# ETM-Code/eirgrid

Hardware: NVIDIA B200
Metric: full 2025-2050 episodes simulated and scored per second (higher is better)
Workload: dtype f64

## Files before the change

### eirgrid_b200/_lib.py

```python
import ctypes as C
import os

import numpy as np

from . import _abi

HERE = os.path.dirname(os.path.abspath(__file__))
LIB_PATH = os.path.join(HERE, os.environ.get("EIRGRID_LIB_NAME", "libeirgrid_b200.so"))

EXPORTS = [
    "eg_init", "eg_destroy", "eg_last_error", "eg_sync", "eg_kernel_launches", "eg_map_load", "eg_map_set",
    "eg_map_info", "eg_map_site_tables", "eg_map_site_static", "eg_weights_new", "eg_weights_free",
    "eg_weights_clone", "eg_weights_load_json", "eg_weights_save_json", "eg_weights_merge", "eg_weights_get_table",
    "eg_weights_set_table", "eg_weights_get_best", "eg_deficit_key_action", "eg_rollout_batch", "eg_weights_upload",
    "eg_rollout_batch_device", "eg_replay_batch", "eg_replay_batch_device", "eg_update", "eg_update_stats_device",
    "eg_update_apply_stats", "eg_location_analysis", "eg_update_stats_clear_device", "eg_update_pack_best_device",
    "eg_location_analysis_year", "eg_microbench_fp64", "eg_export_best_run_csv", "eg_weights_history_append", "eg_train_batch_begin", "eg_train_batch_end", "eg_train_batch_results", "eg_update_combine_apply",
    "eg_update_device", "eg_train_batch_inorder", "eg_rule_math",
    "eg_location_analysis_sites", "eg_location_analysis_sites_device", "eg_location_analysis_write",
    "eg_update_pack_exchange_device",
]


class EirgridError(RuntimeError):
    def __init__(self, code, message):
        super().__init__("eirgrid_b200 error %d: %s" % (code, message))
        self.code = code


_lib = None


def lib():
    global _lib
    if _lib is not None:
        return _lib
    if not os.path.exists(LIB_PATH):
        raise ImportError("%s is missing: run `python -m eirgrid_b200.build` (needs nvcc). "
                          "eirgrid_b200 has no CPU fallback." % LIB_PATH)
    L = C.CDLL(LIB_PATH)
    vp, u32, u64, i64 = C.c_void_p, C.c_uint32, C.c_uint64, C.c_int64
    L.eg_last_error.restype = C.c_char_p
    L.eg_init.argtypes = [C.c_int, vp, C.POINTER(vp)]
# ... 11 lines not shown
    L.eg_weights_free.argtypes = [vp]
    L.eg_weights_free.restype = None
    L.eg_weights_clone.argtypes = [vp, C.POINTER(vp)]
    L.eg_weights_load_json.argtypes = [C.c_char_p, C.POINTER(vp)]
    L.eg_weights_save_json.argtypes = [vp, C.c_char_p]
    L.eg_weights_merge.argtypes = [vp, vp]
    L.eg_weights_get_table.argtypes = [vp, C.POINTER(_abi.WeightsTable)]
    L.eg_weights_set_table.argtypes = [vp, C.POINTER(_abi.WeightsTable)]
    L.eg_weights_get_best.argtypes = [vp, vp, vp, C.c_size_t, vp, vp, C.c_size_t]
    L.eg_deficit_key_action.argtypes = [u32]
    L.eg_deficit_key_action.restype = C.c_uint8
    L.eg_rollout_batch.argtypes = [vp, vp, C.POINTER(_abi.RunCfg), u64, u64, u32, vp, vp, vp, vp]
    L.eg_weights_upload.argtypes = [vp, vp]
    L.eg_rollout_batch_device.argtypes = [vp, C.POINTER(_abi.RunCfg), u64, u64, u32, vp, vp, vp, vp]
    L.eg_replay_batch.argtypes = [vp, C.POINTER(_abi.RunCfg), vp, u32, vp, vp, vp]
    L.eg_replay_batch_device.argtypes = [vp, C.POINTER(_abi.RunCfg), vp, u32, vp, vp, vp]
    L.eg_update.argtypes = [vp, vp, vp, u32, u32, u64, C.POINTER(_abi.UpdateStats)]
    L.eg_update_device.argtypes = [vp, vp, vp, vp, u32, u32, u64, C.POINTER(_abi.UpdateStats)]
    L.eg_train_batch_inorder.argtypes = [vp, vp, C.POINTER(_abi.RunCfg), u64, u64, u32, u64, C.POINTER(_abi.UpdateStats)]
    L.eg_update_stats_device.argtypes = [vp, vp, vp, vp, u32, vp, vp, vp]
    L.eg_update_stats_clear_device.argtypes = [vp, vp]
    L.eg_update_pack_exchange_device.argtypes = [vp, vp, vp, u32, vp, vp, vp, u64, vp, vp, u32, u32, u32, vp]
    L.eg_update_pack_best_device.argtypes = [vp, vp, vp, u32, vp, vp, u64, vp]
    L.eg_weights_history_append.argtypes = [vp, u64, C.c_char_p]
    L.eg_location_analysis_sites.argtypes = [vp, C.c_int, u32, C.c_double, u32, u32, u32, u32, vp]
    L.eg_location_analysis_sites_device.argtypes = [vp, C.c_int, u32, C.c_double, u32, u32, u32, u32, vp]
    L.eg_location_analysis_write.argtypes = [vp, C.c_int, C.c_double, C.c_char_p, C.c_char_p]
    L.eg_rule_math.argtypes = [C.c_int, u32, vp, vp, u32, vp]
    L.eg_microbench_fp64.argtypes = [C.c_int, C.POINTER(C.c_double)]
    L.eg_export_best_run_csv.argtypes = [vp, vp, C.POINTER(_abi.RunCfg), C.c_char_p, C.c_char_p]
    L.eg_train_batch_begin.argtypes = [vp, vp, C.POINTER(_abi.RunCfg), u64, u64, u32]
    L.eg_train_batch_end.argtypes = [vp, vp, vp]
    L.eg_train_batch_results.argtypes = [vp, vp, vp]
    L.eg_update_combine_apply.argtypes = [vp, vp, vp, u32, u64, u64, C.POINTER(_abi.UpdateStats)]
    L.eg_update_apply_stats.argtypes = [vp, vp, u64, vp, vp, i64, C.POINTER(_abi.UpdateStats)]
    L.eg_location_analysis.argtypes = [vp, C.c_int, C.c_int32, C.c_double, vp, u32, u32]
    L.eg_location_analysis_year.argtypes = [vp, C.c_int, u32, C.c_int32, C.c_double, vp, u32, u32]
    _lib = L
    return L


def check(rc):
    if rc < 0:
        raise EirgridError(rc, lib().eg_last_error().decode("utf-8", "replace"))
    return rc

# ... 189 lines not shown
        st = _abi.UpdateStats()
        check(self.L.eg_update_device(self.h, weights.h, _dev_ptr(d_results), _dev_ptr(d_traj), int(n), int(replay_best),
                                      int(rng_seed), C.byref(st)))
        return st

    def train_batch_inorder(self, weights, n, seed, first_episode, cfg=None, rng_seed=0):
        cfg = cfg or _abi.RunCfg()
        st = _abi.UpdateStats()
        check(self.L.eg_train_batch_inorder(self.h, weights.h, C.byref(cfg), int(seed), int(first_episode), int(n),
                                            int(rng_seed), C.byref(st)))
        return st

    def update_stats_device(self, weights, n, d_results, d_traj, d_stats, d_best_score, d_best_index):
        check(self.L.eg_update_stats_device(self.h, weights.h, _dev_ptr(d_results), _dev_ptr(d_traj), n,
                                            _dev_ptr(d_stats), _dev_ptr(d_best_score), _dev_ptr(d_best_index)))

    def update_stats_clear_device(self, d_stats):
        check(self.L.eg_update_stats_clear_device(self.h, _dev_ptr(d_stats)))

    def update_pack_best_device(self, n, d_results, d_traj, d_best_score, d_best_index, first_global_episode, d_record):
        check(self.L.eg_update_pack_best_device(self.h, _dev_ptr(d_results), _dev_ptr(d_traj), n, _dev_ptr(d_best_score),
                                                _dev_ptr(d_best_index), first_global_episode, _dev_ptr(d_record)))

    def update_pack_exchange_device(self, n, d_results, d_traj, d_stats, d_best_score, d_best_index, first_global_episode,
                                    peer_buffers, peer_flags, rank, epoch, d_error):
        world = len(peer_buffers)
        pb = (C.c_uint64 * world)(*[int(x) for x in peer_buffers])
        pf = (C.c_uint64 * world)(*[int(x) for x in peer_flags])
        check(self.L.eg_update_pack_exchange_device(self.h, _dev_ptr(d_results), _dev_ptr(d_traj), n, _dev_ptr(d_stats),
                                                    _dev_ptr(d_best_score), _dev_ptr(d_best_index), int(first_global_episode),
                                                    pb, pf, world, int(rank), int(epoch), _dev_ptr(d_error)))

    def export_best_run_csv(self, weights, output_dir, cfg=None):
        cfg = cfg or _abi.RunCfg()
        buf = C.create_string_buffer(512)
        check(self.L.eg_export_best_run_csv(self.h, weights.h, C.byref(cfg), os.fsencode(output_dir), buf))
        return buf.value.decode()

    def location_analysis(self, use_loaded_map, half_steps=25, step=2000.0, first_point=0, n_points=None, year_index=0):
        side = 2 * half_steps + 1
        n = side * side - first_point if n_points is None else n_points
        out = np.zeros((n, _abi.N_GEN_TYPES))
        check(self.L.eg_location_analysis_year(self.h, int(use_loaded_map), int(year_index), half_steps, step, _abi.ptr(out), first_point, n))
        return out

    def location_analysis_sites(self, use_loaded_map, sites_per_axis, step, year_first=0, n_years=26, first_site=0, n_sites=None,
# ... 28 lines not shown
```

### eirgrid_b200/csrc/engine.cu

```cuda
#include <cuda_runtime.h>
#include <cmath>
#include <sys/stat.h>
#include <sys/types.h>
#include <cstdio>
#include <cstdlib>
#include <cstring>
#include <ctime>
#include <string>
#include <vector>
#include "common.hpp"
#include "episode.cuh"
#include "host_tables.hpp"
#include "json_min.hpp"
#include "site_tables.cuh"
#include "stats.cuh"
#include "suitability.cuh"
#include "update.cuh"
#include "weights.hpp"

static_assert(sizeof(EgPolicyDevice) == 38784, "bench.py and eirgrid_b200/_abi.py quote this size");
static thread_local std::string g_last_error;
int eg_fail(int code, const std::string& message) {
  g_last_error = message;
  return code;
// ... 24 lines not shown
  double* d_prefix = nullptr;
  double* d_static_unsorted = nullptr;
  uint16_t* d_order = nullptr;
  double* d_static_sorted = nullptr;
  double* d_prefix_sorted = nullptr;
  double* d_walk = nullptr;
  double* d_near = nullptr;
  int* d_r2_limit = nullptr;
  double *d_sx = nullptr, *d_sy = nullptr, *d_ex = nullptr, *d_ey = nullptr, *d_cx = nullptr, *d_cy = nullptr;
  uint32_t* d_pop = nullptr;
  double* d_suit_rows = nullptr;
  size_t suit_rows_cap = 0;
  double* d_urban_r = nullptr;
  double urban_r_max = 0.0;
  EgPolicyDevice* d_policy = nullptr;
  EgPolicyDevice* h_policy[2] = {nullptr, nullptr};
  cudaEvent_t policy_copied[2] = {nullptr, nullptr};
  int policy_turn = 0;
  uint32_t* d_next_episode = nullptr;
  int64_t* d_stats = nullptr;
  double* d_best_score = nullptr;
  unsigned long long* d_best_index = nullptr;
  unsigned char* d_record = nullptr;
  int64_t* h_stats = nullptr;
  unsigned char* h_record = nullptr;
  uint32_t train_n = 0;
  bool train_pending = false;
  EgUpdBuffers upd{};
  EgUpdState* h_upd_state = nullptr;
  EgUpdSlot* h_upd_slot = nullptr;
  EgUpdImprovement* h_upd_imp = nullptr;
  EgDeviceMap dmap{};
  size_t cap = 0;
  eg_result* s_out = nullptr;
  eg_traj* s_traj = nullptr;
  eg_traj* s_traj_in = nullptr;
  eg_sites* s_sites = nullptr;
  eg_yearly* s_yearly = nullptr;
  size_t cap_yearly = 0, cap_sites = 0, cap_traj_in = 0;
};

namespace {

void free_map(eg_ctx* c) {
  void* ptrs[] = {c->d_small, c->d_plant_terms, c->d_site_opinion, c->d_coast, c->d_prefix, c->d_static_unsorted, c->d_order,
                  c->d_static_sorted, c->d_prefix_sorted, c->d_walk, c->d_near, c->d_r2_limit, c->d_sx, c->d_sy, c->d_ex, c->d_ey, c->d_cx, c->d_cy, c->d_pop, c->d_urban_r};
// ... 173 lines not shown
  if (e3 != cudaSuccess) { if (c->own_stream) cudaStreamDestroy(c->stream); delete c; return eg_fail(EG_ERR_CUDA, cudaGetErrorString(e3)); }
  *out = c;
  return EG_OK;
}

void eg_destroy(eg_ctx* c) {
  if (!c) return;
  cudaSetDevice(c->device);
  cudaStreamSynchronize(c->stream);
  free_map(c);
  if (c->h_stats) cudaFreeHost(c->h_stats);
  if (c->h_record) cudaFreeHost(c->h_record);
  for (int b = 0; b < 2; b++) {
    if (c->h_policy[b]) cudaFreeHost(c->h_policy[b]);
    if (c->policy_copied[b]) cudaEventDestroy(c->policy_copied[b]);
  }
  if (c->h_upd_state) cudaFreeHost(c->h_upd_state);
  if (c->h_upd_slot) cudaFreeHost(c->h_upd_slot);
  if (c->h_upd_imp) cudaFreeHost(c->h_upd_imp);
  if (c->d_suit_rows) cudaFree(c->d_suit_rows);
  void* upd_ptrs[] = {c->upd.state, c->upd.slots, c->upd.score, c->upd.pre, c->upd.ctl, c->upd.counts, c->upd.factors, c->upd.improvements};
  for (void* p : upd_ptrs)
    if (p) cudaFree(p);
  void* ptrs[] = {c->d_policy, c->d_next_episode, c->d_stats, c->d_best_score, c->d_best_index, c->d_record, c->s_out, c->s_traj, c->s_traj_in, c->s_sites, c->s_yearly};
  for (void* p : ptrs)
    if (p) cudaFree(p);
  if (c->own_stream) cudaStreamDestroy(c->stream);
  delete c;
}

int eg_sync(eg_ctx* c) {
  if (!c) return eg_fail(EG_ERR_INVALID, "ctx is NULL");
  EG_CUDA(cudaStreamSynchronize(c->stream));
  return EG_OK;
}

uint64_t eg_kernel_launches(const eg_ctx* c) { return c ? c->launches : 0; }

int eg_map_load(eg_ctx* c, const char* settlements_json, const char* generators_csv, const char* coastline_json) {
  if (!c || !settlements_json || !generators_csv || !coastline_json) return eg_fail(EG_ERR_INVALID, "eg_map_load: NULL argument");
  int rc = eg_host_map_load(&c->hmap, settlements_json, generators_csv, coastline_json);
  if (rc) return rc;
  return build_device_map(c);
}

int eg_map_set(eg_ctx* c, const eg_map_desc* desc) {
  if (!c) return eg_fail(EG_ERR_INVALID, "eg_map_set: ctx is NULL");
// ... 112 lines not shown
  p.replay_in = d_in;
  p.out = d_out; p.traj = nullptr; p.sites = d_sites; p.yearly = d_yearly;
  EG_CUDA(eg_launch_replay(p, c->stream));
  if (n) c->launches++;
  return EG_OK;
}

int eg_replay_batch(eg_ctx* c, const eg_run_cfg* cfg, const eg_traj* in, uint32_t n, eg_result* out, eg_sites* sites_out,
                    eg_yearly* yearly_out) {
  int rc = check_cfg(c, cfg);
  if (rc) return rc;
  if (!in || !out) return eg_fail(EG_ERR_INVALID, "eg_replay_batch: NULL argument");
  if ((rc = ensure_scratch(c, n, sites_out != nullptr, yearly_out != nullptr, true))) return rc;
  EG_CUDA(cudaMemcpyAsync(c->s_traj_in, in, (size_t)n * sizeof(eg_traj), cudaMemcpyHostToDevice, c->stream));
  rc = eg_replay_batch_device(c, cfg, c->s_traj_in, n, c->s_out, sites_out ? c->s_sites : nullptr, yearly_out ? c->s_yearly : nullptr);
  if (rc) return rc;
  EG_CUDA(cudaMemcpyAsync(out, c->s_out, (size_t)n * sizeof(eg_result), cudaMemcpyDeviceToHost, c->stream));
  if (sites_out) EG_CUDA(cudaMemcpyAsync(sites_out, c->s_sites, (size_t)n * sizeof(eg_sites), cudaMemcpyDeviceToHost, c->stream));
  if (yearly_out) EG_CUDA(cudaMemcpyAsync(yearly_out, c->s_yearly, (size_t)n * sizeof(eg_yearly), cudaMemcpyDeviceToHost, c->stream));
  EG_CUDA(cudaStreamSynchronize(c->stream));
  return EG_OK;
}

int eg_update_stats_device(eg_ctx* c, const eg_weights* w, const eg_result* d_results, const eg_traj* d_trajs, uint32_t n,
                           int64_t* d_stats, double* d_best_score, unsigned long long* d_best_index) {
  if (!c || !w || !d_results || !d_trajs || !d_stats || !d_best_score || !d_best_index)
    return eg_fail(EG_ERR_INVALID, "eg_update_stats_device: NULL argument");
  if (!c->policy_ready) return eg_fail(EG_ERR_STATE, "no weights uploaded: call eg_weights_upload first");
  EG_CUDA(cudaSetDevice(c->device));
  EgStatsParams p{};
  p.consts = eg_contrast_consts(*w);
  p.policy = c->d_policy;
  p.results = d_results; p.trajs = d_trajs; p.n = n;
  p.stats = d_stats; p.best_score = d_best_score; p.best_index = d_best_index;
  p.ln100 = std::log(50000000000.0 * 100.0 / 50000000000.0);
  EG_CUDA(eg_launch_stats(p, c->stream));
  c->launches += n ? 3 : 1;
  return EG_OK;
}

int eg_update_stats_clear_device(eg_ctx* c, int64_t* d_stats) {
  if (!c || !d_stats) return eg_fail(EG_ERR_INVALID, "eg_update_stats_clear_device: NULL argument");
  EG_CUDA(cudaSetDevice(c->device));
  EG_CUDA(cudaMemsetAsync(d_stats, 0, (size_t)EG_STATS_WORDS * sizeof(int64_t), c->stream));
  return EG_OK;
}

int eg_update_pack_best_device(eg_ctx* c, const eg_result* d_results, const eg_traj* d_trajs, uint32_t n, const double* d_best_score,
                               const unsigned long long* d_best_index, uint64_t first_global_episode, void* d_record) {
  if (!c || !d_results || !d_trajs || !d_best_score || !d_best_index || !d_record)
    return eg_fail(EG_ERR_INVALID, "eg_update_pack_best_device: NULL argument");
  EG_CUDA(cudaSetDevice(c->device));
  EG_CUDA(eg_launch_pack_best(d_results, d_trajs, n, d_best_score, d_best_index, first_global_episode, d_record, c->stream));
  c->launches++;
  return EG_OK;
}

int eg_update_pack_exchange_device(eg_ctx* c, const eg_result* d_results, const eg_traj* d_trajs, uint32_t n, const int64_t* d_stats,
                                   const double* d_best_score, const unsigned long long* d_best_index, uint64_t first_global_episode,
                                   const uint64_t* peer_buffers, const uint64_t* peer_flags, uint32_t world, uint32_t rank, uint32_t epoch,
                                   uint32_t* d_error) {
// ... 8 lines not shown
  EG_CUDA(eg_launch_pack_exchange(p, c->stream));
  c->launches++;
  return EG_OK;
}

int eg_train_batch_begin(eg_ctx* c, const eg_weights* w, const eg_run_cfg* cfg, uint64_t seed, uint64_t first_episode, uint32_t n) {
  int rc = check_cfg(c, cfg);
  if (rc) return rc;
  if (!w) return eg_fail(EG_ERR_INVALID, "eg_train_batch_begin: weights are NULL");
  if (c->train_pending) return eg_fail(EG_ERR_STATE, "eg_train_batch_begin: a batch is already in flight on this context");
  EG_CUDA(cudaSetDevice(c->device));
  if (!c->d_stats) {
    EG_CUDA(cudaMalloc((void**)&c->d_stats, EG_STATS_WORDS * sizeof(int64_t)));
    EG_CUDA(cudaMalloc((void**)&c->d_best_score, sizeof(double)));
    EG_CUDA(cudaMalloc((void**)&c->d_best_index, sizeof(unsigned long long)));
    EG_CUDA(cudaMalloc((void**)&c->d_record, EG_BEST_RECORD_BYTES));
    EG_CUDA(cudaMallocHost((void**)&c->h_stats, EG_STATS_WORDS * sizeof(int64_t)));
    EG_CUDA(cudaMallocHost((void**)&c->h_record, EG_BEST_RECORD_BYTES));
  }
  if ((rc = eg_weights_upload(c, w))) return rc;
  if ((rc = ensure_scratch(c, n, false, false, false))) return rc;
  if ((rc = eg_rollout_batch_device(c, cfg, seed, first_episode, n, c->s_out, c->s_traj, nullptr, nullptr))) return rc;
  if ((rc = eg_update_stats_clear_device(c, c->d_stats))) return rc;
  if ((rc = eg_update_stats_device(c, w, c->s_out, c->s_traj, n, c->d_stats, c->d_best_score, c->d_best_index))) return rc;
  if ((rc = eg_update_pack_best_device(c, c->s_out, c->s_traj, n, c->d_best_score, c->d_best_index, first_episode, c->d_record))) return rc;
  EG_CUDA(cudaMemcpyAsync(c->h_stats, c->d_stats, EG_STATS_WORDS * sizeof(int64_t), cudaMemcpyDeviceToHost, c->stream));
  EG_CUDA(cudaMemcpyAsync(c->h_record, c->d_record, EG_BEST_RECORD_BYTES, cudaMemcpyDeviceToHost, c->stream));
  c->train_n = n;
  c->train_pending = true;
  return EG_OK;
}

int eg_train_batch_end(eg_ctx* c, int64_t* stats_out, void* record_out) {
  if (!c || !stats_out || !record_out) return eg_fail(EG_ERR_INVALID, "eg_train_batch_end: NULL argument");
  if (!c->train_pending) return eg_fail(EG_ERR_STATE, "eg_train_batch_end: no batch in flight");
  EG_CUDA(cudaSetDevice(c->device));
  c->train_pending = false;
  EG_CUDA(cudaStreamSynchronize(c->stream));
  std::memcpy(stats_out, c->h_stats, EG_STATS_WORDS * sizeof(int64_t));
  std::memcpy(record_out, c->h_record, EG_BEST_RECORD_BYTES);
  return EG_OK;
}

int eg_train_batch_results(eg_ctx* c, eg_result* out, eg_traj* traj_out) {
  if (!c || !out) return eg_fail(EG_ERR_INVALID, "eg_train_batch_results: NULL argument");
  if (c->train_pending || !c->train_n) return eg_fail(EG_ERR_STATE, "eg_train_batch_results: no finished batch");
  EG_CUDA(cudaSetDevice(c->device));
  EG_CUDA(cudaMemcpyAsync(out, c->s_out, (size_t)c->train_n * sizeof(eg_result), cudaMemcpyDeviceToHost, c->stream));
// ... 534 lines not shown
```

### eirgrid_b200/csrc/stats.cu

```cuda
#include "stats.cuh"
#include <algorithm>

namespace {

constexpr double kMaxAcceptableCost = 50000000000.0, kMaxAcceptableEmissions = 1000000.0;

__device__ __forceinline__ double default_score(const eg_result& r, double ln100, bool cost_only = false) {
  if (cost_only) return 2.0 - fmin(log(fmax(r.total_cost / kMaxAcceptableCost, 1.0)) / ln100, 1.0);
  if (r.net_emissions > 0.0) return 1.0 - fmin(r.net_emissions / kMaxAcceptableEmissions, 1.0);
  const double normalized_cost = fmax(r.total_cost / kMaxAcceptableCost, 1.0);
  const double cost_score = 1.0 - fmin(log(normalized_cost) / ln100, 1.0);
  const double cost_weight = normalized_cost > 8.0 ? 0.8 : 0.5;
  return 1.0 + (cost_score * cost_weight + r.public_opinion * (1.0 - cost_weight));
}

__device__ __forceinline__ int deficit_key_of_action(int code) {
  if (code == EG_ACT_DO_NOTHING) return 14;
  if (code >= 45 || code % 3) return -1;
  switch (code / 3) {
    case 8: return 0; case 7: return 1; case 12: return 2; case 11: return 3; case 9: return 4; case 0: return 5;
    case 1: return 6; case 4: return 7; case 10: return 8; case 5: return 9; case 2: return 10; case 3: return 11;
    case 13: return 12; case 14: return 13;
  }
  return -1;
}

__global__ void eg_stats_reset_kernel(double* best_score, unsigned long long* best_index) {
  *best_score = -1.0;
  *best_index = ~0ull;
}

__global__ void __launch_bounds__(256) eg_stats_kernel(const EgStatsParams p) {
  __shared__ unsigned long long acc[EG_STATS_WORDS];
  __shared__ unsigned long long best_mask[EG_NY];
  __shared__ uint8_t best_cat[EG_BEST_CAPACITY + EG_TRAJ_CAPACITY];
  __shared__ uint16_t best_len[EG_NY], best_start[EG_NY];
  for (int i = threadIdx.x; i < EG_STATS_WORDS; i += blockDim.x) acc[i] = 0ull;
  if (threadIdx.x < EG_NY) {
    const int y = threadIdx.x;
    const int nb = p.policy->n_best[y], nbd = p.policy->n_best_deficit[y];
    const int ob = p.policy->best_off[y], obd = p.policy->best_deficit_off[y];
    uint8_t* cat = best_cat + ob + obd;
    unsigned long long m = 0ull;
    for (int b = 0; b < nb; b++) { const int a = p.policy->best[ob + b]; cat[b] = (uint8_t)a; m |= 1ull << a; }
    for (int b = 0; b < nbd; b++) { const int a = p.policy->best_deficit[obd + b]; cat[nb + b] = (uint8_t)a; m |= 1ull << a; }
    best_mask[y] = m;
    best_len[y] = (uint16_t)(nb + nbd);
    best_start[y] = (uint16_t)(ob + obd);
  }
  __syncthreads();
  const int lane = threadIdx.x & 31;
  const uint32_t warps_total = gridDim.x * (blockDim.x >> 5);
  double warp_best = -1.0;
  for (uint32_t ep = blockIdx.x * (blockDim.x >> 5) + (threadIdx.x >> 5); ep < p.n; ep += warps_total) {
    const eg_result* rp = p.results + ep;
    eg_result r;
    r.net_emissions = rp->net_emissions; r.public_opinion = rp->public_opinion; r.total_cost = rp->total_cost;
    const double score = default_score(r, p.ln100, p.consts.cost_only != 0);
    warp_best = fmax(warp_best, score);
    bool pass = false;
    long long log_pen = 0, log_mild = 0;
    if (p.consts.has_best) {
      const double det = p.consts.best_score > 0.0 ? (p.consts.best_score - score) / p.consts.best_score : 0.0;
      pass = det > p.consts.threshold || p.consts.force;
      if (pass) {
        if (det < 0.0) {
          log_pen = log_mild = -(1ll << 40);
        } else {
          const double combined = pow(det, 0.3) * p.consts.stagnation;
          const double penalty = 1.0 / (1.0 + p.consts.alr * 1.5 * combined);
          const double mild = 1.0 / (1.0 + p.consts.alr * combined * 0.5);
          log_pen = llrint(log(penalty) * EG_STATS_FIXED_SCALE);
          log_mild = llrint(log(mild) * EG_STATS_FIXED_SCALE);
        }
      }
    }
    if (lane == 0) {
      atomicAdd(&acc[0], 1ull);
      if (pass) atomicAdd(&acc[1], 1ull);
      if (rp->flags) atomicAdd(&acc[2], 1ull);
    }
    const eg_traj* t = p.trajs + ep;
    int nd = 0, nrun = 0;
    if (lane < EG_NY) { nd = t->n_deficit[lane]; nrun = nd + t->n_additional[lane]; }
    int row_end = nrun;
#pragma unroll
    for (int o = 1; o < 32; o <<= 1) {
      const int v = __shfl_up_sync(0xFFFFFFFFu, row_end, o);
      if (lane >= o) row_end += v;
    }
    int row = row_end - nrun;
    if (row > EG_TRAJ_CAPACITY) row = EG_TRAJ_CAPACITY;
    if (row + nrun > EG_TRAJ_CAPACITY) { nrun = EG_TRAJ_CAPACITY - row; nd = min(nd, nrun); }
    const int cnt = nrun + nd;
    int incl = cnt;
#pragma unroll
    for (int o = 1; o < 32; o <<= 1) {
      const int v = __shfl_up_sync(0xFFFFFFFFu, incl, o);
      if (lane >= o) incl += v;
    }
    const int total = __shfl_sync(0xFFFFFFFFu, incl, 31);
    for (int base = 0; base < total; base += 32) {
      const int q = base + lane;
      int y = 0;
#pragma unroll
      for (int step = 16; step > 0; step >>= 1) {
        const int v = __shfl_sync(0xFFFFFFFFu, incl, y + step - 1);
        if (v <= q) y += step;
      }
      const int y_incl = __shfl_sync(0xFFFFFFFFu, incl, y), y_cnt = __shfl_sync(0xFFFFFFFFu, cnt, y);
      const int y_nrun = __shfl_sync(0xFFFFFFFFu, nrun, y), y_row = __shfl_sync(0xFFFFFFFFu, row, y);
      if (q >= total) continue;
      const int i = q - (y_incl - y_cnt);
      const int a = t->actions[y_row + (i < y_nrun ? i : i - y_nrun)];
      if (a >= EG_N_ACTIONS) continue;
      unsigned long long* ys = acc + EG_STATS_HEADER + y * EG_STATS_YEAR_STRIDE;
      if (i < y_nrun) atomicAdd(&ys[2 * EG_N_ACTIONS + a], 1ull);
      else {
        const int k = deficit_key_of_action(a);
        if (k >= 0) atomicAdd(&ys[3 * EG_N_ACTIONS + k], 1ull);
      }
      if (!pass) continue;
      if (!((best_mask[y] >> a) & 1ull)) {
        atomicAdd(&ys[a], (unsigned long long)log_pen);
      } else if (i < (int)best_len[y]) {
        if (best_cat[best_start[y] + i] != a) atomicAdd(&ys[EG_N_ACTIONS + a], (unsigned long long)log_mild);
      }
    }
  }
  if (lane == 0 && warp_best >= 0.0) atomicMax((long long*)p.best_score, __double_as_longlong(warp_best));
  __syncthreads();
  for (int i = threadIdx.x; i < EG_STATS_WORDS; i += blockDim.x)
    if (acc[i]) atomicAdd((unsigned long long*)&p.stats[i], acc[i]);
}

__global__ void __launch_bounds__(256) eg_stats_argbest_kernel(const EgStatsParams p) {
  const uint32_t ep = blockIdx.x * blockDim.x + threadIdx.x;
  if (ep >= p.n) return;
  const double score = default_score(p.results[ep], p.ln100, p.consts.cost_only != 0);
  if (score == *p.best_score) atomicMin(p.best_index, (unsigned long long)ep);
}

__global__ void __launch_bounds__(320) eg_stats_pack_best_kernel(const eg_result* results, const eg_traj* trajs, uint32_t n, const double* best_score,
                                                                 const unsigned long long* best_index, unsigned long long first_global, uint32_t* record) {
  const unsigned long long raw = *best_index;
  const uint32_t idx = raw < n ? (uint32_t)raw : (n ? n - 1 : 0);
  const int w = threadIdx.x;
  constexpr int kRes = (int)sizeof(eg_result) / 4, kTraj = (int)sizeof(eg_traj) / 4;
  if (w < 2) record[w] = ((const uint32_t*)best_score)[w];
  else if (w < 4) { const unsigned long long g = first_global + idx; record[w] = (uint32_t)(g >> (32 * (w - 2))); }
  else if (w < 4 + kRes) record[w] = ((const uint32_t*)(results + idx))[w - 4];
  else if (w < 4 + kRes + kTraj) record[w] = ((const uint32_t*)(trajs + idx))[w - 4 - kRes];
}

__global__ void __launch_bounds__(256) eg_pack_exchange_kernel(const EgExchangeParams p) {
  constexpr int kRec = (int)(EG_BEST_RECORD_BYTES / 8), kWords = EG_STATS_WORDS + kRec;
  constexpr int kRes = (int)sizeof(eg_result) / 8;
  const uint32_t peer = blockIdx.x;
  const unsigned long long raw = *p.best_index;
  const uint32_t idx = raw < p.n ? (uint32_t)raw : (p.n ? p.n - 1 : 0);
  long long* dst = (long long*)p.peer_buf[peer] + ((size_t)(p.epoch & 1u) * p.world + p.rank) * kWords;
  const long long* res = (const long long*)(p.results + idx);
  const long long* trj = (const long long*)(p.trajs + idx);
  for (int i = threadIdx.x; i < kWords; i += blockDim.x) {
    long long v;
    if (i < EG_STATS_WORDS) v = p.stats[i];
    else {
      const int w = i - EG_STATS_WORDS;
      v = w == 0 ? __double_as_longlong(*p.best_score) : w == 1 ? (long long)(p.first_global + idx) : w < 2 + kRes ? res[w - 2] : trj[w - 2 - kRes];
    }
    dst[i] = v;
  }
  __threadfence_system();
  __syncthreads();
  if (threadIdx.x == 0) {
// ... 6 lines not shown
      asm volatile("ld.acquire.sys.global.u32 %0, [%1];" : "=r"(v) : "l"(mine) : "memory");
      if ((int32_t)(v - p.epoch) >= 0) break;
      if (clock64() - t0 > 4000000000ll) { *p.error = 1u; break; }
    }
  }
}

}

cudaError_t eg_launch_pack_exchange(const EgExchangeParams& p, cudaStream_t stream) {
  static_assert(EG_BEST_RECORD_BYTES % 8 == 0 && sizeof(eg_result) % 8 == 0 && sizeof(eg_traj) % 8 == 0, "the record is copied in 64-bit words");
  if (p.world == 0 || p.world > EG_MAX_PEERS || p.rank >= p.world) return cudaErrorInvalidValue;
  eg_pack_exchange_kernel<<<p.world, 256, 0, stream>>>(p);
  return cudaGetLastError();
}

cudaError_t eg_launch_pack_best(const eg_result* results, const eg_traj* trajs, uint32_t n, const double* best_score,
                                const unsigned long long* best_index, unsigned long long first_global, void* record, cudaStream_t stream) {
  static_assert(sizeof(eg_result) % 4 == 0 && sizeof(eg_traj) % 4 == 0, "record is copied in 32-bit words");
  eg_stats_pack_best_kernel<<<1, 320, 0, stream>>>(results, trajs, n, best_score, best_index, first_global, (uint32_t*)record);
  return cudaGetLastError();
}

cudaError_t eg_launch_stats(const EgStatsParams& p, cudaStream_t stream) {
  eg_stats_reset_kernel<<<1, 1, 0, stream>>>(p.best_score, p.best_index);
  if (p.n == 0) return cudaGetLastError();
  const uint32_t blocks = (p.n + 255) / 256;
  int dev = 0, sms = 148;
  cudaGetDevice(&dev);
  cudaDeviceGetAttribute(&sms, cudaDevAttrMultiProcessorCount, dev);
  const uint32_t stat_blocks = std::min<uint32_t>((uint32_t)sms * 4u, (p.n + 7) / 8);
  eg_stats_kernel<<<stat_blocks, 256, 0, stream>>>(p);
  eg_stats_argbest_kernel<<<blocks, 256, 0, stream>>>(p);
  return cudaGetLastError();
}
```

### eirgrid_b200/csrc/stats.cuh

```cuda
#pragma once
#include <cuda_runtime.h>
#include "tables.h"
#include "weights.hpp"

struct EgStatsParams {
  EgContrastConsts consts;
  const EgPolicyDevice* policy;
  const eg_result* results;
  const eg_traj* trajs;
  uint32_t n;
  int64_t* stats;
  double* best_score;
  unsigned long long* best_index;
  double ln100;
};

cudaError_t eg_launch_pack_best(const eg_result* results, const eg_traj* trajs, uint32_t n, const double* best_score,
                                const unsigned long long* best_index, unsigned long long first_global, void* record, cudaStream_t stream);

cudaError_t eg_launch_stats(const EgStatsParams& p, cudaStream_t stream);

#define EG_MAX_PEERS 16
struct EgExchangeParams {
  const eg_result* results;
  const eg_traj* trajs;
  uint32_t n;
  const double* best_score;
  const unsigned long long* best_index;
  unsigned long long first_global;
  const int64_t* stats;
  unsigned long long peer_buf[EG_MAX_PEERS];
  unsigned long long peer_flag[EG_MAX_PEERS];
  uint32_t world, rank, epoch;
  uint32_t* error;
};
cudaError_t eg_launch_pack_exchange(const EgExchangeParams& p, cudaStream_t stream);
```

### eirgrid_b200/trainer.py

```python
import ctypes as C
import os

import numpy as np

from . import _abi, _lib


def _torch():
    import torch
    return torch


REC_BYTES = 16 + _abi.RESULT_DTYPE.itemsize + _abi.TRAJ_DTYPE.itemsize
assert REC_BYTES % 8 == 0


def pack_record(score, global_index, result, traj):
    rec = np.zeros(REC_BYTES, np.uint8)
    rec[0:8] = np.frombuffer(np.float64(score).tobytes(), np.uint8)
    rec[8:16] = np.frombuffer(np.int64(global_index).tobytes(), np.uint8)
    rb = _abi.RESULT_DTYPE.itemsize
    rec[16:16 + rb] = np.frombuffer(np.ascontiguousarray(result).tobytes(), np.uint8)
    rec[16 + rb:] = np.frombuffer(np.ascontiguousarray(traj).tobytes(), np.uint8)
    return rec
# ... 48 lines not shown
        assert self.stream.cuda_stream != 0
        if map_arrays is not None:
            self.ctx.map_set(*map_arrays)
        else:
            self.ctx.map_load_dir(asset_dir)
        self.n = int(episodes_per_gpu)
        self.seed = int(seed)
        self.cfg = cfg or _abi.RunCfg()
        self.weights = weights or _lib.Weights()
        self.next_episode = 0
        self.offset = self.rank * self.n
        self.n_total = self.n * self.world
        u8 = torch.uint8
        self.d_results = torch.empty(self.n * _abi.RESULT_DTYPE.itemsize, dtype=u8, device=self.device)
        self.d_traj = torch.empty(self.n * _abi.TRAJ_DTYPE.itemsize, dtype=u8, device=self.device)
        self.d_sites = torch.empty(self.n * _abi.SITES_DTYPE.itemsize, dtype=u8, device=self.device) if want_sites else None
        self.rec_bytes = REC_BYTES
        self.pack_words = PACK_WORDS
        self.d_pack = torch.zeros(self.pack_words, dtype=torch.int64, device=self.device)
        self.d_stats = self.d_pack[:_abi.STATS_WORDS]
        self.d_rec = self.d_pack[_abi.STATS_WORDS:].view(u8)
        self.d_best_score = torch.zeros(1, dtype=torch.float64, device=self.device)
        self.d_best_index = torch.zeros(1, dtype=torch.int64, device=self.device)
        self.d_all_pack = torch.zeros(self.world * self.pack_words, dtype=torch.int64, device=self.device)
        self.h_all_pack = torch.zeros(self.world * self.pack_words, dtype=torch.int64).pin_memory()
        self.h2d_bytes_per_step = 0
        self.d2h_bytes_per_step = self.h_all_pack.numel() * 8
        self._init_peer_exchange()
        self.last_stats = None
        torch.cuda.synchronize(self.device)

    def _init_peer_exchange(self):
        torch = _torch()
        self.peer = None
        self.exchange_kind = "none" if self.world == 1 else "nccl all-gather"
        if not (self.dist and self.world > 1):
            return
        ok, peer = 1, None
        if os.environ.get("EIRGRID_EXCHANGE", "peer") != "peer":
            ok = 0
        else:
            try:
                import torch.distributed._symmetric_memory as symm
                buf = symm.empty(2 * self.world * self.pack_words, dtype=torch.int64, device=self.device)
                hdl = symm.rendezvous(buf, self.dist.group.WORLD)
                flags = symm.empty(64, dtype=torch.int32, device=self.device)
                fhdl = symm.rendezvous(flags, self.dist.group.WORLD)
# ... 11 lines not shown
        torch.cuda.synchronize(self.device)
        if int(agree.item()) == 1:
            self.peer = peer
            self.epoch = 0
            self.d_error = torch.zeros(1, dtype=torch.int32, device=self.device)
            self.exchange_kind = "one kernel over NVLink peer memory (symmetric allocation)"
            self.dist.barrier()
            torch.cuda.synchronize(self.device)

    def set_batch(self, total):
        self.offset, self.n = shard_of(total, self.rank, self.world)
        assert self.n <= self.d_results.numel() // _abi.RESULT_DTYPE.itemsize, "batch larger than the buffers"
        self.n_total = int(total)

    def upload_weights(self):
        self.ctx.weights_upload(self.weights)

    def launch_rollout(self, first_episode=None):
        first = self.next_episode + self.offset if first_episode is None else first_episode
        self.ctx.rollout_device(self.n, self.seed, first, self.d_results, self.d_traj, self.d_sites, None, self.cfg)

    def launch_stats(self):
        self.ctx.update_stats_clear_device(self.d_stats)
        self.ctx.update_stats_device(self.weights, self.n, self.d_results, self.d_traj, self.d_stats, self.d_best_score,
                                     self.d_best_index)

    def _pack_best(self):
        self.ctx.update_pack_best_device(self.n, self.d_results, self.d_traj, self.d_best_score, self.d_best_index,
                                         self.next_episode + self.offset, self.d_rec)

    def exchange(self):
        if self.peer is not None:
            self.epoch += 1
            self.ctx.update_pack_exchange_device(self.n, self.d_results, self.d_traj, self.d_stats, self.d_best_score, self.d_best_index,
                                                 self.next_episode + self.offset, self.peer["buf_ptrs"], self.peer["flag_ptrs"], self.rank,
                                                 self.epoch, self.d_error)
            half = (self.epoch & 1) * self.world * self.pack_words
            self.d_all_pack = self.peer["buf"][half:half + self.world * self.pack_words]
            return
        self._pack_best()
        with _torch().cuda.stream(self.stream):
            if self.dist and self.world > 1:
                self.dist.all_gather_into_tensor(self.d_all_pack, self.d_pack)
            else:
                self.d_all_pack.copy_(self.d_pack)

    def reduce_stats(self):
        self.exchange()

    def check_exchange(self):
        if self.peer is not None and int(self.d_error.item()) != 0:
            raise _lib.EirgridError(-3, "exchange step: a peer rank did not deliver its statistics within 2 s")

    def warm_exchange(self):
        self.exchange()
        with _torch().cuda.stream(self.stream):
            self.h_all_pack.copy_(self.d_all_pack, non_blocking=True)
        self.stream.synchronize()

    def step(self):
        torch = _torch()
        self.upload_weights()
        self.launch_rollout()
        self.launch_stats()
        self.exchange()
        with torch.cuda.stream(self.stream):
            self.h_all_pack.copy_(self.d_all_pack, non_blocking=True)
        self.stream.synchronize()
# ... 51 lines not shown
```

### include/eirgrid_b200.h

```cpp
#ifndef EIRGRID_B200_H
#define EIRGRID_B200_H

#include <stddef.h>
#include <stdint.h>

#ifdef __cplusplus
extern "C" {
#endif

#define EG_BASE_YEAR 2025
#define EG_END_YEAR 2050
#define EG_N_YEARS 26
#define EG_N_GEN_TYPES 15
#define EG_N_OFFSET_TYPES 4
#define EG_N_MULTS 3
#define EG_N_ACTIONS 61
#define EG_N_DEFICIT_KEYS 15
#define EG_N_COUNT_KEYS 21
#define EG_TRAJ_CAPACITY 984
#define EG_BEST_CAPACITY (2 * EG_TRAJ_CAPACITY)
#define EG_SITE_NONE 0xFFFFu

#define EG_ACT_UPGRADE 57
#define EG_ACT_ADJUST 58
// ... 158 lines not shown
int eg_replay_batch(eg_ctx* ctx, const eg_run_cfg* cfg, const eg_traj* in, uint32_t n, eg_result* out,
                    eg_sites* sites_out, eg_yearly* yearly_out);
int eg_replay_batch_device(eg_ctx* ctx, const eg_run_cfg* cfg, const eg_traj* d_in, uint32_t n,
                           eg_result* d_out, eg_sites* d_sites, eg_yearly* d_yearly);

int eg_update(eg_weights* w, const eg_result* results, const eg_traj* trajs, uint32_t n,
              uint32_t replay_best, uint64_t rng_seed, eg_update_stats* stats_out);

int eg_update_device(eg_ctx* ctx, eg_weights* w, const eg_result* d_results, const eg_traj* d_trajs, uint32_t n,
                     uint32_t replay_best, uint64_t rng_seed, eg_update_stats* stats_out);
int eg_train_batch_inorder(eg_ctx* ctx, eg_weights* w, const eg_run_cfg* cfg, uint64_t seed, uint64_t first_episode, uint32_t n,
                           uint64_t rng_seed, eg_update_stats* stats_out);

#define EG_STATS_WORDS (8 + EG_N_YEARS * (3 * EG_N_ACTIONS + EG_N_DEFICIT_KEYS))
int eg_update_stats_device(eg_ctx* ctx, const eg_weights* w, const eg_result* d_results, const eg_traj* d_trajs, uint32_t n,
                           int64_t* d_stats ,
                           double* d_best_score ,
                           unsigned long long* d_best_index );
int eg_update_stats_clear_device(eg_ctx* ctx, int64_t* d_stats);
#define EG_BEST_RECORD_BYTES (16 + sizeof(eg_result) + sizeof(eg_traj))
int eg_update_pack_best_device(eg_ctx* ctx, const eg_result* d_results, const eg_traj* d_trajs, uint32_t n,
                               const double* d_best_score, const unsigned long long* d_best_index,
                               uint64_t first_global_episode, void* d_record);
int eg_update_pack_exchange_device(eg_ctx* ctx, const eg_result* d_results, const eg_traj* d_trajs, uint32_t n, const int64_t* d_stats,
                                   const double* d_best_score, const unsigned long long* d_best_index, uint64_t first_global_episode,
                                   const uint64_t* peer_buffers, const uint64_t* peer_flags, uint32_t world, uint32_t rank,
                                   uint32_t epoch, uint32_t* d_error);
int eg_update_apply_stats(eg_weights* w, const int64_t* stats, uint64_t n_total,
                          const eg_result* batch_best_result, const eg_traj* batch_best_traj,
                          int64_t batch_best_index, eg_update_stats* stats_out);

int eg_train_batch_begin(eg_ctx* ctx, const eg_weights* w, const eg_run_cfg* cfg, uint64_t seed, uint64_t first_episode, uint32_t n);
int eg_train_batch_end(eg_ctx* ctx, int64_t* stats_out, void* record_out);
int eg_train_batch_results(eg_ctx* ctx, eg_result* out, eg_traj* traj_out );
int eg_update_combine_apply(eg_weights* w, const int64_t* stats_sum, const void* records, uint32_t n_records,
                            uint64_t n_total, uint64_t first_episode, eg_update_stats* stats_out);

int eg_export_best_run_csv(eg_ctx* ctx, const eg_weights* w, const eg_run_cfg* cfg, const char* output_dir, char* written_dir);

int eg_location_analysis(eg_ctx* ctx, int use_loaded_map, int32_t half_steps, double step,
                         double* scores_out, uint32_t first_point, uint32_t n_points);
int eg_location_analysis_year(eg_ctx* ctx, int use_loaded_map, uint32_t year_index, int32_t half_steps, double step,
                              double* scores_out, uint32_t first_point, uint32_t n_points);

int eg_location_analysis_sites(eg_ctx* ctx, int use_loaded_map, uint32_t sites_per_axis, double step, uint32_t year_first,
                               uint32_t n_years, uint32_t first_site, uint32_t n_sites, double* scores_out);
// ... 12 lines not shown
```

Measured before the change: 20.43 million.

## Fuse stats reset, argbest and best-record packing into one stats kernel

Replaces the reset, stats and argbest kernels plus the separate pack-best kernel with a single stats kernel. It tracks per-warp best score and index, reduces them per block, and uses a last-block ticket to pick the global best and write the record. It also prefetches the next episode's loads, reads actions through warp shuffles of a preloaded word, and skips the single-GPU device copy of the pack buffer. The cost removed is several launches and full extra passes over results. In exchange it adds a grid-wide ticket that relies on threadfence ordering and a persistent scratch buffer.

New measurement: 20.51 million (median of 6 runs). Within noise of the previous version (+0.4%).

```diff
diff --git a/eirgrid_b200/_lib.py b/eirgrid_b200/_lib.py
--- a/eirgrid_b200/_lib.py
+++ b/eirgrid_b200/_lib.py
@@ -18,7 +18,7 @@
     "eg_location_analysis_year", "eg_microbench_fp64", "eg_export_best_run_csv", "eg_weights_history_append", "eg_train_batch_begin", "eg_train_batch_end", "eg_train_batch_results", "eg_update_combine_apply",
     "eg_update_device", "eg_train_batch_inorder", "eg_rule_math",
     "eg_location_analysis_sites", "eg_location_analysis_sites_device", "eg_location_analysis_write",
-    "eg_update_pack_exchange_device",
+    "eg_update_pack_exchange_device", "eg_update_stats_pack_device",
 ]
 
 
@@ -76,6 +76,7 @@
     L.eg_update_stats_clear_device.argtypes = [vp, vp]
     L.eg_update_pack_exchange_device.argtypes = [vp, vp, vp, u32, vp, vp, vp, u64, vp, vp, u32, u32, u32, vp]
     L.eg_update_pack_best_device.argtypes = [vp, vp, vp, u32, vp, vp, u64, vp]
+    L.eg_update_stats_pack_device.argtypes = [vp, vp, vp, vp, u32, vp, vp, vp, u64, vp]
     L.eg_weights_history_append.argtypes = [vp, u64, C.c_char_p]
     L.eg_location_analysis_sites.argtypes = [vp, C.c_int, u32, C.c_double, u32, u32, u32, u32, vp]
     L.eg_location_analysis_sites_device.argtypes = [vp, C.c_int, u32, C.c_double, u32, u32, u32, u32, vp]
@@ -311,6 +312,12 @@
         check(self.L.eg_update_pack_best_device(self.h, _dev_ptr(d_results), _dev_ptr(d_traj), n, _dev_ptr(d_best_score),
                                                 _dev_ptr(d_best_index), first_global_episode, _dev_ptr(d_record)))
 
+    def update_stats_pack_device(self, weights, n, d_results, d_traj, d_stats, d_best_score, d_best_index, first_global_episode,
+                                 d_record):
+        check(self.L.eg_update_stats_pack_device(self.h, weights.h, _dev_ptr(d_results), _dev_ptr(d_traj), n, _dev_ptr(d_stats),
+                                                 _dev_ptr(d_best_score), _dev_ptr(d_best_index), first_global_episode,
+                                                 _dev_ptr(d_record)))
+
     def update_pack_exchange_device(self, n, d_results, d_traj, d_stats, d_best_score, d_best_index, first_global_episode,
                                     peer_buffers, peer_flags, rank, epoch, d_error):
         world = len(peer_buffers)
diff --git a/eirgrid_b200/csrc/engine.cu b/eirgrid_b200/csrc/engine.cu
--- a/eirgrid_b200/csrc/engine.cu
+++ b/eirgrid_b200/csrc/engine.cu
@@ -70,6 +70,7 @@
   double* d_best_score = nullptr;
   unsigned long long* d_best_index = nullptr;
   unsigned char* d_record = nullptr;
+  unsigned long long* d_stats_scratch = nullptr;
   int64_t* h_stats = nullptr;
   unsigned char* h_record = nullptr;
   uint32_t train_n = 0;
@@ -289,7 +290,7 @@
   void* upd_ptrs[] = {c->upd.state, c->upd.slots, c->upd.score, c->upd.pre, c->upd.ctl, c->upd.counts, c->upd.factors, c->upd.improvements};
   for (void* p : upd_ptrs)
     if (p) cudaFree(p);
-  void* ptrs[] = {c->d_policy, c->d_next_episode, c->d_stats, c->d_best_score, c->d_best_index, c->d_record, c->s_out, c->s_traj, c->s_traj_in, c->s_sites, c->s_yearly};
+  void* ptrs[] = {c->d_policy, c->d_next_episode, c->d_stats, c->d_best_score, c->d_best_index, c->d_record, c->d_stats_scratch, c->s_out, c->s_traj, c->s_traj_in, c->s_sites, c->s_yearly};
   for (void* p : ptrs)
     if (p) cudaFree(p);
   if (c->own_stream) cudaStreamDestroy(c->stream);
@@ -448,21 +449,42 @@
   return EG_OK;
 }
 
-int eg_update_stats_device(eg_ctx* c, const eg_weights* w, const eg_result* d_results, const eg_traj* d_trajs, uint32_t n,
-                           int64_t* d_stats, double* d_best_score, unsigned long long* d_best_index) {
-  if (!c || !w || !d_results || !d_trajs || !d_stats || !d_best_score || !d_best_index)
-    return eg_fail(EG_ERR_INVALID, "eg_update_stats_device: NULL argument");
+static int launch_stats(eg_ctx* c, const eg_weights* w, const eg_result* d_results, const eg_traj* d_trajs, uint32_t n, int64_t* d_stats,
+                        double* d_best_score, unsigned long long* d_best_index, uint64_t first_global_episode, void* d_record) {
   if (!c->policy_ready) return eg_fail(EG_ERR_STATE, "no weights uploaded: call eg_weights_upload first");
   EG_CUDA(cudaSetDevice(c->device));
+  if (!c->d_stats_scratch) {
+    size_t words = 0;
+    EG_CUDA(eg_stats_scratch_words(&words));
+    EG_CUDA(cudaMalloc((void**)&c->d_stats_scratch, words * sizeof(unsigned long long)));
+    EG_CUDA(cudaMemsetAsync(c->d_stats_scratch, 0, words * sizeof(unsigned long long), c->stream));
+  }
   EgStatsParams p{};
   p.consts = eg_contrast_consts(*w);
   p.policy = c->d_policy;
   p.results = d_results; p.trajs = d_trajs; p.n = n;
   p.stats = d_stats; p.best_score = d_best_score; p.best_index = d_best_index;
   p.ln100 = std::log(50000000000.0 * 100.0 / 50000000000.0);
+  p.first_global = first_global_episode; p.record = (uint32_t*)d_record;
+  p.scratch = c->d_stats_scratch;
   EG_CUDA(eg_launch_stats(p, c->stream));
-  c->launches += n ? 3 : 1;
-  return EG_OK;
+  c->launches++;
+  return EG_OK;
+}
+
+int eg_update_stats_device(eg_ctx* c, const eg_weights* w, const eg_result* d_results, const eg_traj* d_trajs, uint32_t n,
+                           int64_t* d_stats, double* d_best_score, unsigned long long* d_best_index) {
+  if (!c || !w || !d_results || !d_trajs || !d_stats || !d_best_score || !d_best_index)
+    return eg_fail(EG_ERR_INVALID, "eg_update_stats_device: NULL argument");
+  return launch_stats(c, w, d_results, d_trajs, n, d_stats, d_best_score, d_best_index, 0, nullptr);
+}
+
+int eg_update_stats_pack_device(eg_ctx* c, const eg_weights* w, const eg_result* d_results, const eg_traj* d_trajs, uint32_t n,
+                                int64_t* d_stats, double* d_best_score, unsigned long long* d_best_index, uint64_t first_global_episode,
+                                void* d_record) {
+  if (!c || !w || !d_results || !d_trajs || !d_stats || !d_best_score || !d_best_index || !d_record)
+    return eg_fail(EG_ERR_INVALID, "eg_update_stats_pack_device: NULL argument");
+  return launch_stats(c, w, d_results, d_trajs, n, d_stats, d_best_score, d_best_index, first_global_episode, d_record);
 }
 
 int eg_update_stats_clear_device(eg_ctx* c, int64_t* d_stats) {
@@ -517,8 +539,8 @@
   if ((rc = ensure_scratch(c, n, false, false, false))) return rc;
   if ((rc = eg_rollout_batch_device(c, cfg, seed, first_episode, n, c->s_out, c->s_traj, nullptr, nullptr))) return rc;
   if ((rc = eg_update_stats_clear_device(c, c->d_stats))) return rc;
-  if ((rc = eg_update_stats_device(c, w, c->s_out, c->s_traj, n, c->d_stats, c->d_best_score, c->d_best_index))) return rc;
-  if ((rc = eg_update_pack_best_device(c, c->s_out, c->s_traj, n, c->d_best_score, c->d_best_index, first_episode, c->d_record))) return rc;
+  if ((rc = eg_update_stats_pack_device(c, w, c->s_out, c->s_traj, n, c->d_stats, c->d_best_score, c->d_best_index, first_episode,
+                                        c->d_record))) return rc;
   EG_CUDA(cudaMemcpyAsync(c->h_stats, c->d_stats, EG_STATS_WORDS * sizeof(int64_t), cudaMemcpyDeviceToHost, c->stream));
   EG_CUDA(cudaMemcpyAsync(c->h_record, c->d_record, EG_BEST_RECORD_BYTES, cudaMemcpyDeviceToHost, c->stream));
   c->train_n = n;
diff --git a/eirgrid_b200/csrc/stats.cu b/eirgrid_b200/csrc/stats.cu
--- a/eirgrid_b200/csrc/stats.cu
+++ b/eirgrid_b200/csrc/stats.cu
@@ -2,6 +2,8 @@
 #include <algorithm>
 
 namespace {
+
+constexpr int kStatsThreads = 256, kStatsBlocksPerSm = 4, kTicketWords = 2;
 
 constexpr double kMaxAcceptableCost = 50000000000.0, kMaxAcceptableEmissions = 1000000.0;
 
@@ -25,16 +27,33 @@
   return -1;
 }
 
-__global__ void eg_stats_reset_kernel(double* best_score, unsigned long long* best_index) {
-  *best_score = -1.0;
-  *best_index = ~0ull;
-}
-
-__global__ void __launch_bounds__(256) eg_stats_kernel(const EgStatsParams p) {
+__device__ __forceinline__ bool better(double s, unsigned long long i, double bs, unsigned long long bi) {
+  return s > bs || (s == bs && i < bi);
+}
+
+__device__ __forceinline__ void write_record(const eg_result* results, const eg_traj* trajs, uint32_t n, double score,
+                                             unsigned long long raw, unsigned long long first_global, uint32_t* record, int t, int nt) {
+  constexpr int kRes = (int)sizeof(eg_result) / 4, kTraj = (int)sizeof(eg_traj) / 4;
+  const uint32_t idx = raw < n ? (uint32_t)raw : (n ? n - 1 : 0);
+  const unsigned long long bits = (unsigned long long)__double_as_longlong(score), g = first_global + idx;
+  for (int w = t; w < 4 + kRes + kTraj; w += nt) {
+    uint32_t v;
+    if (w < 2) v = (uint32_t)(bits >> (32 * w));
+    else if (w < 4) v = (uint32_t)(g >> (32 * (w - 2)));
+    else if (w < 4 + kRes) v = ((const uint32_t*)(results + idx))[w - 4];
+    else v = ((const uint32_t*)(trajs + idx))[w - 4 - kRes];
+    record[w] = v;
+  }
+}
+
+__global__ void __launch_bounds__(kStatsThreads, kStatsBlocksPerSm) eg_stats_kernel(const EgStatsParams p) {
   __shared__ unsigned long long acc[EG_STATS_WORDS];
   __shared__ unsigned long long best_mask[EG_NY];
   __shared__ uint8_t best_cat[EG_BEST_CAPACITY + EG_TRAJ_CAPACITY];
   __shared__ uint16_t best_len[EG_NY], best_start[EG_NY];
+  __shared__ double warp_best_s[kStatsThreads / 32];
+  __shared__ unsigned long long warp_best_i[kStatsThreads / 32];
+  __shared__ int last;
   for (int i = threadIdx.x; i < EG_STATS_WORDS; i += blockDim.x) acc[i] = 0ull;
   if (threadIdx.x < EG_NY) {
     const int y = threadIdx.x;
@@ -49,15 +68,33 @@
     best_start[y] = (uint16_t)(ob + obd);
   }
   __syncthreads();
-  const int lane = threadIdx.x & 31;
+  const int lane = threadIdx.x & 31, warp = threadIdx.x >> 5;
   const uint32_t warps_total = gridDim.x * (blockDim.x >> 5);
   double warp_best = -1.0;
-  for (uint32_t ep = blockIdx.x * (blockDim.x >> 5) + (threadIdx.x >> 5); ep < p.n; ep += warps_total) {
+  unsigned long long warp_best_ep = ~0ull;
+  struct Loads {
+    double net, opinion, cost;
+    uint32_t flags, act4;
+    int nd, nadd;
+  };
+  const auto load = [&](uint32_t ep, Loads& l) {
     const eg_result* rp = p.results + ep;
+    const eg_traj* t = p.trajs + ep;
+    l.net = rp->net_emissions; l.opinion = rp->public_opinion; l.cost = rp->total_cost; l.flags = rp->flags;
+    l.act4 = ((const uint32_t*)t->actions)[lane];
+    l.nd = lane < EG_NY ? t->n_deficit[lane] : 0;
+    l.nadd = lane < EG_NY ? t->n_additional[lane] : 0;
+  };
+  uint32_t ep = blockIdx.x * (blockDim.x >> 5) + warp;
+  Loads cur{};
+  if (ep < p.n) load(ep, cur);
+  for (; ep < p.n; ep += warps_total) {
+    Loads next{};
+    if (ep + warps_total < p.n) load(ep + warps_total, next);
     eg_result r;
-    r.net_emissions = rp->net_emissions; r.public_opinion = rp->public_opinion; r.total_cost = rp->total_cost;
+    r.net_emissions = cur.net; r.public_opinion = cur.opinion; r.total_cost = cur.cost;
     const double score = default_score(r, p.ln100, p.consts.cost_only != 0);
-    warp_best = fmax(warp_best, score);
+    if (score > warp_best) { warp_best = score; warp_best_ep = ep; }
     bool pass = false;
     long long log_pen = 0, log_mild = 0;
     if (p.consts.has_best) {
@@ -78,11 +115,9 @@
     if (lane == 0) {
       atomicAdd(&acc[0], 1ull);
       if (pass) atomicAdd(&acc[1], 1ull);
-      if (rp->flags) atomicAdd(&acc[2], 1ull);
-    }
-    const eg_traj* t = p.trajs + ep;
-    int nd = 0, nrun = 0;
-    if (lane < EG_NY) { nd = t->n_deficit[lane]; nrun = nd + t->n_additional[lane]; }
+      if (cur.flags) atomicAdd(&acc[2], 1ull);
+    }
+    int nd = cur.nd, nrun = cur.nd + cur.nadd;
     int row_end = nrun;
 #pragma unroll
     for (int o = 1; o < 32; o <<= 1) {
@@ -110,9 +145,11 @@
       }
       const int y_incl = __shfl_sync(0xFFFFFFFFu, incl, y), y_cnt = __shfl_sync(0xFFFFFFFFu, cnt, y);
       const int y_nrun = __shfl_sync(0xFFFFFFFFu, nrun, y), y_row = __shfl_sync(0xFFFFFFFFu, row, y);
+      const int i = q - (y_incl - y_cnt);
+      const int slot = q < total ? y_row + (i < y_nrun ? i : i - y_nrun) : 0;
+      const uint32_t word = __shfl_sync(0xFFFFFFFFu, cur.act4, (slot >> 2) & 31);
       if (q >= total) continue;
-      const int i = q - (y_incl - y_cnt);
-      const int a = t->actions[y_row + (i < y_nrun ? i : i - y_nrun)];
+      const int a = slot < 128 ? (int)((word >> (8 * (slot & 3))) & 0xFFu) : p.trajs[ep].actions[slot];
       if (a >= EG_N_ACTIONS) continue;
       unsigned long long* ys = acc + EG_STATS_HEADER + y * EG_STATS_YEAR_STRIDE;
       if (i < y_nrun) atomicAdd(&ys[2 * EG_N_ACTIONS + a], 1ull);
@@ -127,30 +164,57 @@
         if (best_cat[best_start[y] + i] != a) atomicAdd(&ys[EG_N_ACTIONS + a], (unsigned long long)log_mild);
       }
     }
-  }
-  if (lane == 0 && warp_best >= 0.0) atomicMax((long long*)p.best_score, __double_as_longlong(warp_best));
+    cur = next;
+  }
+  if (lane == 0) { warp_best_s[warp] = warp_best; warp_best_i[warp] = warp_best_ep; }
+
   __syncthreads();
   for (int i = threadIdx.x; i < EG_STATS_WORDS; i += blockDim.x)
     if (acc[i]) atomicAdd((unsigned long long*)&p.stats[i], acc[i]);
-}
-
-__global__ void __launch_bounds__(256) eg_stats_argbest_kernel(const EgStatsParams p) {
-  const uint32_t ep = blockIdx.x * blockDim.x + threadIdx.x;
-  if (ep >= p.n) return;
-  const double score = default_score(p.results[ep], p.ln100, p.consts.cost_only != 0);
-  if (score == *p.best_score) atomicMin(p.best_index, (unsigned long long)ep);
+  unsigned int* ticket = (unsigned int*)p.scratch;
+  unsigned long long* block_best = p.scratch + kTicketWords;
+  if (threadIdx.x == 0) {
+    double bs = warp_best_s[0];
+    unsigned long long bi = warp_best_i[0];
+    for (int w = 1; w < kStatsThreads / 32; w++)
+      if (better(warp_best_s[w], warp_best_i[w], bs, bi)) { bs = warp_best_s[w]; bi = warp_best_i[w]; }
+    block_best[2 * blockIdx.x] = (unsigned long long)__double_as_longlong(bs);
+    block_best[2 * blockIdx.x + 1] = bi;
+    __threadfence();
+    last = atomicAdd(ticket, 1u) == gridDim.x - 1;
+  }
+  __syncthreads();
+  if (!last) return;
+  __threadfence();
+  if (warp == 0) {
+    double bs = -1.0;
+    unsigned long long bi = ~0ull;
+    for (uint32_t b = lane; b < gridDim.x; b += 32) {
+      const double s = __longlong_as_double((long long)__ldcg(block_best + 2 * b));
+      const unsigned long long i = __ldcg(block_best + 2 * b + 1);
+      if (better(s, i, bs, bi)) { bs = s; bi = i; }
+    }
+#pragma unroll
+    for (int o = 16; o > 0; o >>= 1) {
+      const double s = __shfl_xor_sync(0xFFFFFFFFu, bs, o);
+      const unsigned long long i = __shfl_xor_sync(0xFFFFFFFFu, bi, o);
+      if (better(s, i, bs, bi)) { bs = s; bi = i; }
+    }
+    if (lane == 0) {
+      *p.best_score = bs;
+      *p.best_index = bi;
+      warp_best_s[0] = bs;
+      warp_best_i[0] = bi;
+    }
+    if (lane == 0) *ticket = 0u;
+  }
+  __syncthreads();
+  if (p.record) write_record(p.results, p.trajs, p.n, warp_best_s[0], warp_best_i[0], p.first_global, p.record, threadIdx.x, blockDim.x);
 }
 
 __global__ void __launch_bounds__(320) eg_stats_pack_best_kernel(const eg_result* results, const eg_traj* trajs, uint32_t n, const double* best_score,
                                                                  const unsigned long long* best_index, unsigned long long first_global, uint32_t* record) {
-  const unsigned long long raw = *best_index;
-  const uint32_t idx = raw < n ? (uint32_t)raw : (n ? n - 1 : 0);
-  const int w = threadIdx.x;
-  constexpr int kRes = (int)sizeof(eg_result) / 4, kTraj = (int)sizeof(eg_traj) / 4;
-  if (w < 2) record[w] = ((const uint32_t*)best_score)[w];
-  else if (w < 4) { const unsigned long long g = first_global + idx; record[w] = (uint32_t)(g >> (32 * (w - 2))); }
-  else if (w < 4 + kRes) record[w] = ((const uint32_t*)(results + idx))[w - 4];
-  else if (w < 4 + kRes + kTraj) record[w] = ((const uint32_t*)(trajs + idx))[w - 4 - kRes];
+  write_record(results, trajs, n, *best_score, *best_index, first_global, record, threadIdx.x, blockDim.x);
 }
 
 __global__ void __launch_bounds__(256) eg_pack_exchange_kernel(const EgExchangeParams p) {
@@ -203,15 +267,24 @@
   return cudaGetLastError();
 }
 
-cudaError_t eg_launch_stats(const EgStatsParams& p, cudaStream_t stream) {
-  eg_stats_reset_kernel<<<1, 1, 0, stream>>>(p.best_score, p.best_index);
-  if (p.n == 0) return cudaGetLastError();
-  const uint32_t blocks = (p.n + 255) / 256;
+namespace {
+
+uint32_t max_blocks() {
   int dev = 0, sms = 148;
   cudaGetDevice(&dev);
   cudaDeviceGetAttribute(&sms, cudaDevAttrMultiProcessorCount, dev);
-  const uint32_t stat_blocks = std::min<uint32_t>((uint32_t)sms * 4u, (p.n + 7) / 8);
-  eg_stats_kernel<<<stat_blocks, 256, 0, stream>>>(p);
-  eg_stats_argbest_kernel<<<blocks, 256, 0, stream>>>(p);
+  return (uint32_t)sms * kStatsBlocksPerSm;
+}
+
+}
+
+cudaError_t eg_stats_scratch_words(size_t* words) {
+  *words = kTicketWords + 2 * (size_t)max_blocks();
+  return cudaSuccess;
+}
+
+cudaError_t eg_launch_stats(const EgStatsParams& p, cudaStream_t stream) {
+  const uint32_t blocks = std::max(1u, std::min(max_blocks(), (p.n + kStatsThreads / 32 - 1) / (kStatsThreads / 32)));
+  eg_stats_kernel<<<blocks, kStatsThreads, 0, stream>>>(p);
   return cudaGetLastError();
 }
diff --git a/eirgrid_b200/csrc/stats.cuh b/eirgrid_b200/csrc/stats.cuh
--- a/eirgrid_b200/csrc/stats.cuh
+++ b/eirgrid_b200/csrc/stats.cuh
@@ -13,10 +13,15 @@
   double* best_score;
   unsigned long long* best_index;
   double ln100;
+  unsigned long long first_global;
+  uint32_t* record;
+  unsigned long long* scratch;
 };
 
 cudaError_t eg_launch_pack_best(const eg_result* results, const eg_traj* trajs, uint32_t n, const double* best_score,
                                 const unsigned long long* best_index, unsigned long long first_global, void* record, cudaStream_t stream);
+
+cudaError_t eg_stats_scratch_words(size_t* words);
 
 cudaError_t eg_launch_stats(const EgStatsParams& p, cudaStream_t stream);
 
diff --git a/eirgrid_b200/trainer.py b/eirgrid_b200/trainer.py
--- a/eirgrid_b200/trainer.py
+++ b/eirgrid_b200/trainer.py
@@ -94,7 +94,7 @@
         self.d_rec = self.d_pack[_abi.STATS_WORDS:].view(u8)
         self.d_best_score = torch.zeros(1, dtype=torch.float64, device=self.device)
         self.d_best_index = torch.zeros(1, dtype=torch.int64, device=self.device)
-        self.d_all_pack = torch.zeros(self.world * self.pack_words, dtype=torch.int64, device=self.device)
+        self.d_all_pack = self.d_pack if self.world == 1 else torch.zeros(self.world * self.pack_words, dtype=torch.int64, device=self.device)
         self.h_all_pack = torch.zeros(self.world * self.pack_words, dtype=torch.int64).pin_memory()
         self.h2d_bytes_per_step = 0
         self.d2h_bytes_per_step = self.h_all_pack.numel() * 8
@@ -152,12 +152,8 @@
 
     def launch_stats(self):
         self.ctx.update_stats_clear_device(self.d_stats)
-        self.ctx.update_stats_device(self.weights, self.n, self.d_results, self.d_traj, self.d_stats, self.d_best_score,
-                                     self.d_best_index)
-
-    def _pack_best(self):
-        self.ctx.update_pack_best_device(self.n, self.d_results, self.d_traj, self.d_best_score, self.d_best_index,
-                                         self.next_episode + self.offset, self.d_rec)
+        self.ctx.update_stats_pack_device(self.weights, self.n, self.d_results, self.d_traj, self.d_stats, self.d_best_score,
+                                          self.d_best_index, self.next_episode + self.offset, self.d_rec)
 
     def exchange(self):
         if self.peer is not None:
@@ -168,12 +164,9 @@
             half = (self.epoch & 1) * self.world * self.pack_words
             self.d_all_pack = self.peer["buf"][half:half + self.world * self.pack_words]
             return
-        self._pack_best()
-        with _torch().cuda.stream(self.stream):
-            if self.dist and self.world > 1:
+        if self.world > 1:
+            with _torch().cuda.stream(self.stream):
                 self.dist.all_gather_into_tensor(self.d_all_pack, self.d_pack)
-            else:
-                self.d_all_pack.copy_(self.d_pack)
 
     def reduce_stats(self):
         self.exchange()
diff --git a/include/eirgrid_b200.h b/include/eirgrid_b200.h
--- a/include/eirgrid_b200.h
+++ b/include/eirgrid_b200.h
@@ -204,6 +204,9 @@
 int eg_update_pack_best_device(eg_ctx* ctx, const eg_result* d_results, const eg_traj* d_trajs, uint32_t n,
                                const double* d_best_score, const unsigned long long* d_best_index,
                                uint64_t first_global_episode, void* d_record);
+int eg_update_stats_pack_device(eg_ctx* ctx, const eg_weights* w, const eg_result* d_results, const eg_traj* d_trajs, uint32_t n,
+                                int64_t* d_stats, double* d_best_score, unsigned long long* d_best_index,
+                                uint64_t first_global_episode, void* d_record);
 int eg_update_pack_exchange_device(eg_ctx* ctx, const eg_result* d_results, const eg_traj* d_trajs, uint32_t n, const int64_t* d_stats,
                                    const double* d_best_score, const unsigned long long* d_best_index, uint64_t first_global_episode,
                                    const uint64_t* peer_buffers, const uint64_t* peer_flags, uint32_t world, uint32_t rank,
```
